# OpenVisualCloud/SVT-VP9

Hardware: AMD Instinct MI355X
Metric: hot-path frames/sec (+ Mpixels/sec): block-level DSP path (picture analysis + ME + inter prediction from reconstructed references + DCT/quant/recon + deblock + reference padding), 3840x2160p60 yuv420p enc-mode 8; no mode decision, no entropy coding -- not encoded frames (higher is better)
Workload: dtype u8

## Files before the change

### include/svtvp9_hip.h

```cpp
#ifndef SVTVP9_HIP_H
#define SVTVP9_HIP_H

#include <stddef.h>
#include <stdint.h>

#ifdef __cplusplus
extern "C" {
#endif

typedef enum svt_hip_status {
    SVT_HIP_OK                 = 0,
    SVT_HIP_ERR_BAD_PARAMETER  = -1,
    SVT_HIP_ERR_NO_RESOURCES   = -2,
    SVT_HIP_ERR_DEVICE         = -3,
    SVT_HIP_ERR_UNSUPPORTED    = -4
} svt_hip_status;

typedef struct svt_hip_ctx svt_hip_ctx;


#define SVT_ME_PU_COUNT 85
#define SVT_SB_SIZE 64

typedef struct svt_plane {
// ... 63 lines not shown

typedef struct svt_me_picture_config {
    int32_t pic_width, pic_height;
    int32_t enc_mode;
    int32_t tune;
    int32_t frame_rate;
    int32_t num_ref_lists;
    int32_t temporal_layer_index;
    int32_t hierarchical_levels;
    int32_t is_used_as_reference;
    int32_t same_ref_poc;
    int32_t rate_control_mode;
} svt_me_picture_config;

int32_t svt_hip_me_params_derive(svt_me_params *p, const svt_me_picture_config *cfg);

int32_t svt_hip_me_params_preset(svt_me_params *p, int32_t pic_width, int32_t pic_height, int32_t enc_mode,
                                 int32_t tune, int32_t num_ref_lists, int32_t temporal_layer_index,
                                 int32_t hierarchical_levels);

int32_t svt_hip_me_kernel_instance(const svt_me_params *p);
int32_t svt_hip_me_last_instance(const svt_hip_ctx *ctx);
int32_t svt_hip_me_lds_bytes(const svt_me_params *p, int32_t compact);
int32_t svt_hip_ctx_set_intra_workgroups(svt_hip_ctx *ctx, int32_t n);
int32_t svt_hip_ctx_warm(svt_hip_ctx *ctx);
int32_t svt_hip_ctx_warm_scratch(svt_hip_ctx *ctx, int32_t scratch_bytes);
int32_t svt_hip_me_params_same_launch(const svt_me_params *a, const svt_me_params *b);

int32_t svt_hip_ctx_create(svt_hip_ctx **ctx, int32_t device_ordinal);
int32_t svt_hip_ctx_create_on_stream(svt_hip_ctx **ctx, int32_t device_ordinal, void *hip_stream);
int32_t svt_hip_ctx_create_cu_mask(svt_hip_ctx **ctx, int32_t device, const uint32_t *cu_mask, int32_t mask_words);
void *svt_hip_ctx_stream(svt_hip_ctx *ctx);
void    svt_hip_ctx_destroy(svt_hip_ctx *ctx);
int32_t svt_hip_ctx_synchronize(svt_hip_ctx *ctx);
const char *svt_hip_last_error(void);
float   svt_hip_last_kernel_ms(svt_hip_ctx *ctx);

int32_t svt_hip_mem_alloc(svt_hip_ctx *ctx, size_t bytes, void **d_ptr);
void    svt_hip_mem_free(svt_hip_ctx *ctx, void *d_ptr);
int32_t svt_hip_mem_upload_2d(svt_hip_ctx *ctx, void *d_dst, size_t dst_stride, const void *src, size_t src_stride, size_t width_bytes,
                              size_t rows);
int32_t svt_hip_mem_download(svt_hip_ctx *ctx, void *dst, const void *d_src, size_t bytes);
int32_t svt_hip_mem_upload_2d_async(svt_hip_ctx *ctx, void *d_dst, size_t dst_stride, const void *src, size_t src_stride, size_t width_bytes,
                                    size_t rows);
int32_t svt_hip_mem_upload_planes_async(svt_hip_ctx *ctx, int32_t n_planes, void *const *d_dst, const size_t *dst_stride, const void *const *src,
                                        const size_t *src_stride, const size_t *width_bytes, const size_t *rows);
// ... 625 lines not shown
```

### svt-vp9_amd/binding.py

```python
import ctypes as C
import os

import numpy as np

HERE = os.path.dirname(os.path.abspath(__file__))
LIB_PATH = os.environ.get("SVT_HIP_LIB") or os.path.join(HERE, "libsvtvp9_hip.so")

SVT_ME_PU_COUNT = 85


class Plane(C.Structure):
    _fields_ = [("buf", C.c_void_p), ("stride", C.c_int32), ("origin_x", C.c_int32), ("origin_y", C.c_int32),
                ("width", C.c_int32), ("height", C.c_int32)]


class PaPicture(C.Structure):
    _fields_ = [("full", Plane), ("quarter", Plane), ("sixteenth", Plane)]


class MeParams(C.Structure):
    _fields_ = [(n, C.c_uint8) for n in (
        "num_ref_lists", "temporal_layer_index", "hierarchical_levels", "enable_hme_flag",
        "enable_hme_level_0_flag", "enable_hme_level_1_flag", "enable_hme_level_2_flag", "cu8x8_mode",
        "cu16x16_mode", "same_ref_poc", "rate_control_mode", "fractional_search_method",
# ... 210 lines not shown
OIS_BLOCK_DTYPE = np.dtype([("sad", "<u4"), ("uv_sad", "<u4"), ("mode", "u1"), ("uv_mode", "u1"), ("pad", "u1", (2,))])
assert OIS_BLOCK_DTYPE.itemsize == 12
OIS_PER_SB = 340
OIS_NONE = 0xFFFFFFFF

EXPORTS = [
    "svt_hip_sb_count", "svt_hip_input_resolution", "svt_hip_me_params_derive", "svt_hip_me_params_preset", "svt_hip_ctx_create", "svt_hip_ctx_create_on_stream", "svt_hip_ctx_create_cu_mask", "svt_hip_ctx_stream",
    "svt_hip_ctx_destroy", "svt_hip_ctx_synchronize", "svt_hip_last_error", "svt_hip_last_kernel_ms",
    "svt_hip_mem_alloc", "svt_hip_mem_free", "svt_hip_mem_upload_2d", "svt_hip_mem_upload_2d_async", "svt_hip_mem_upload_planes_async", "svt_hip_mem_download", "svt_hip_mem_set",
    "svt_hip_ctx_marker_record", "svt_hip_ctx_marker_query", "svt_hip_ctx_marker_wait", "svt_hip_minigop_split",
    "svt_hip_me_picture_device", "svt_hip_me_batch_device", "svt_hip_me_batch_layers_device", "svt_hip_me_picture", "svt_hip_sad_loop_batch_device",
    "svt_hip_me_zz_sad_device", "svt_hip_me_similar_collocated", "svt_hip_me_sb_stats_device", "svt_hip_pa_prepare_batch_device", "svt_hip_pa_mean_variance_device",
    "svt_hip_quant_tables_init", "svt_hip_tq_batch_device", "svt_hip_tq_batch_dist_device", "svt_hip_tq_rd_batch_device", "svt_hip_tq_rd_batch_multi_device", "svt_hip_rate_scan4x4_table", "svt_hip_tq_batch", "svt_hip_lf_thresh_init", "svt_hip_lf_level_from_q",
    "svt_hip_lf_frame_device", "svt_hip_lf_batch_device", "svt_hip_lf_frame", "svt_hip_lf_build_masks",
    "svt_hip_inter_pred_batch_device", "svt_hip_inter_pred_frame", "svt_hip_ref_pad_batch_device", "svt_hip_coeff_rate_batch_device", "svt_hip_coeff_rate_batch",
    "svt_hip_gop_owner", "svt_hip_gop_assign", "svt_hip_minigop_reference_source", "svt_hip_device_set_create", "svt_hip_device_set_size",
    "svt_hip_device_set_ctx", "svt_hip_device_set_destroy", "svt_hip_ref_handoff_device",
    "svt_ivf_stream_header", "svt_ivf_packetize",
    "svt_hip_tq_blocks_from_grid", "svt_hip_vp9_iscan_tables", "svt_hip_vp9_qindex_from_qp", "svt_hip_vp9_dc_step", "svt_hip_vp9_ac_step",
    "svt_hip_quant_tables_for_qindex", "svt_hip_encdec_flags_derive", "svt_hip_encdec_work_create", "svt_hip_encdec_work_destroy",
    "svt_hip_encdec_batch_device", "svt_hip_encdec_intra_device", "svt_hip_md_intra_default_device", "svt_hip_encdec_work_status", "svt_hip_encdec_work_download", "svt_hip_md_default_batch_device",
    "svt_hip_md_default_picture", "svt_hip_lf_build_masks_device", "svt_hip_ctx_wait_marker", "svt_hip_host_alloc", "svt_hip_host_free",
    "svt_hip_mem_download_2d_async", "svt_hip_mem_copy_2d_device", "svt_hip_encdec_work_set_stage_hook", "svt_hip_me_params_same_launch", "svt_hip_me_kernel_instance", "svt_hip_ctx_set_intra_workgroups", "svt_hip_ctx_warm", "svt_hip_ctx_warm_scratch", "svt_hip_lf_reserve",
    "svt_hip_me_last_instance", "svt_hip_me_lds_bytes", "svt_hip_vp9_layer_qindex", "svt_hip_mem_upload_2d_direct", "svt_hip_mem_upload_wait", "svt_hip_host_unregister_all", "svt_hip_host_registry_retain", "svt_hip_host_registry_release",
    "svt_hip_intra_search_device", "svt_hip_md_intra_search_device", "svt_hip_md_intra_search_picture",
    "svt_hip_pa_noise_params_derive", "svt_hip_pa_noise_batch_device", "svt_hip_pa_histogram_batch_device", "svt_hip_pa_chroma_mean_batch_device",
    "svt_hip_vp9_scan_tables", "svt_hip_tokenize_blocks_device", "svt_hip_tokenize_blocks", "svt_hip_tokenize_blocks_host", "svt_hip_tokenize_batch_device", "svt_hip_tokenize_picture",
    "svt_hip_tokenize_capacity",
    "svt_hip_boolcode_set_tables", "svt_hip_boolcode_batch_device", "svt_hip_boolcode", "svt_hip_boolcode_host", "svt_hip_boolcode_capacity", "svt_hip_boolcode_bools_capacity",
    "svt_hip_boolcode_geometry",
    "svt_hip_modes_set_tables", "svt_hip_modes_kf_batch_device", "svt_hip_modes_kf_picture", "svt_hip_modes_segments", "svt_hip_modes_bools_capacity",
    "svt_hip_modes_inter_set_tables", "svt_hip_modes_inter_batch_device", "svt_hip_modes_inter_picture", "svt_hip_modes_inter_bools_capacity",
    "svt_hip_mvrefs_batch_device", "svt_hip_mvrefs_picture",
    "svt_hip_md_inter_modes_batch_device", "svt_hip_md_inter_modes_picture",
    "svt_hip_frame_header_host", "svt_hip_frame_show_existing_host", "svt_hip_frame_batch_device", "svt_hip_frame_assemble_host", "svt_hip_frame_geometry",
]

_lib = None


def load():
    global _lib
    if _lib is None:
        if not os.path.exists(LIB_PATH):
            raise RuntimeError(f"{LIB_PATH} not built: run `python -c 'import __graft_entry__ as g; g.build()'`")
        try:
            import torch
# ... 84 lines not shown
```

### svt-vp9_amd/csrc/intra_kernel.hip

```cpp
#include <hip/hip_runtime.h>
#include "tq_core.h"
#include "encdec_core.h"
#include "intra_pred.h"
#include <stdlib.h>

namespace {

struct intra_pic_dev {
    const uint8_t *src[3];
    uint8_t       *pred[3];
    uint8_t       *rec[3];
    int32_t        src_stride[2], pred_stride[2], rec_stride[2];
    const svt_lf_mode_info *mi;
    int32_t        mi_stride, mi_rows, mi_cols, sb_cols, sb_rows, width, height;
    const svt_quant_tables *qtabs;
    const int16_t *iscan;
    uint32_t       iscan_off[16];
    int16_t       *qcoeff, *dqcoeff;
    uint16_t      *eob_map;
    uint8_t       *nz;
    int32_t       *sync;
    int32_t       *status;
    int32_t        mixed;
};

#ifdef INTRA_FENCES
#define INTRA_WT false
#define INTRA_LD(p) (*(p))
#else
#define INTRA_WT true
#define INTRA_LD(p) __hip_atomic_load((p), __ATOMIC_RELAXED, __HIP_MEMORY_SCOPE_AGENT)
#endif
#ifdef INTRA_PROF
__device__ unsigned long long g_intra_fine[8];
#define IPF(k) do { if (lane == 0) { const unsigned long long n_ = __builtin_amdgcn_s_memtime(); atomicAdd(&g_intra_fine[k], n_ - ipf_t); ipf_t = n_; } } while (0)
#else
#define IPF(k) ((void)0)
#endif
#define INTRA_TILE_DW  (2 * 32 * 33)
#define INTRA_SLICE_DW (INTRA_TILE_DW + 128 / 4)
#define INTRA_W        4
template <int N>
__device__ __forceinline__ int intra_block(const intra_pic_dev &P, int plane, int x0, int y0, int mode, int sb, int32_t *lds, int have_right = 0) {
    const int lane = (int)__lane_id(), c = plane ? 1 : 0;
    int32_t *const tile = lds + __builtin_amdgcn_readfirstlane((int)threadIdx.x >> 6) * INTRA_SLICE_DW;
    uint8_t *const edge = (uint8_t *)(tile + INTRA_TILE_DW);
    const int rs = P.rec_stride[c];
    uint8_t  *rp = P.rec[plane];
    const int have_left = x0 > 0, have_top = y0 > 0;
    const bool active = lane < N;
    const int  i = lane % N;
#ifdef INTRA_PROF
    unsigned long long ipf_t = __builtin_amdgcn_s_memtime();
#endif
    uint32_t   srow[N / 4], prow[N / 4];
    constexpr uintptr_t AM = N >= 16 ? 15 : N - 1;
    {
        const uint8_t *sp = P.src[plane] + (size_t)(y0 + i) * P.src_stride[c] + x0;
        _Pragma("unroll") for (int q = 0; q < N / 4; q++) srow[q] = 0u;
        if (active) row_load<N>(sp, ((uintptr_t)sp & AM) == 0, srow);
    }
    {
// ... 11 lines not shown
        if (lane == 0) edge[32] = have_top ? (have_left ? INTRA_LD(&rp[(size_t)(y0 - 1) * rs + x0 - 1]) : (uint8_t)129) : (uint8_t)127;
    }
    tq_block_sync();
    IPF(0);
    intra_pred_row<N>(edge, mode, i, have_left, have_top, prow);
    {
        if (active && P.pred[plane]) {
            uint8_t *pp = P.pred[plane] + (size_t)(y0 + i) * P.pred_stride[c] + x0;
            row_store<N>(pp, ((uintptr_t)pp & AM) == 0, prow);
        }
    }
    IPF(1);
    svt_tq_block k;
    k.src_off = k.pred_off = 0;
    k.recon_off = (uint32_t)y0 * (uint32_t)rs + (uint32_t)x0;
    k.coeff_off = (uint32_t)sb * SVT_SB_COEFFS + (plane == 0 ? 0u : plane == 1 ? 4096u : 5120u) + svt_zorder4((x0 & (plane ? 31 : 63)) >> 2, (y0 & (plane ? 31 : 63)) >> 2) * 16u;
    k.tx_size = (uint8_t)txcfg<N>::size;
    k.tx_type = (uint8_t)((plane == 0 && N < 32) ? intra_tx_type(mode) : 0);
    k.iscan_off = P.iscan_off[k.tx_size * 4 + k.tx_type];
    k.src_stride = k.pred_stride = 0; k.recon_stride = (uint16_t)rs;
    k.qtab = (uint8_t)c; k.do_recon = 1; k.partial32 = 0; k.pad_[0] = 0;
    const int pw4 = (plane ? P.width >> 1 : P.width) >> 2, w4 = P.width >> 2, h4 = P.height >> 2;
    const int eo = plane == 0 ? 0 : w4 * h4 + (plane == 2 ? (w4 >> 1) * (h4 >> 1) : 0);
    int32_t *t = tile + (lane / N) * (N * (N + 1));
    const int eob = tq_block_body<N, false, false, INTRA_WT>(k, active, i, t, srow, prow, P.qtabs, P.iscan, P.qcoeff, P.dqcoeff,
                                                   P.eob_map + eo + (y0 >> 2) * pw4 + (x0 >> 2), nullptr, nullptr, nullptr, nullptr, nullptr, rp);
    IPF(2);
    __builtin_amdgcn_fence(__ATOMIC_SEQ_CST, "workgroup");
    tq_block_sync();
    IPF(3);
    return __builtin_amdgcn_readfirstlane(eob);
}

#ifndef INTRA_WAVES_PER_EU
#define INTRA_WAVES_PER_EU 4
#endif
#ifdef INTRA_NUM_VGPR
__attribute__((amdgpu_num_vgpr(INTRA_NUM_VGPR)))
#endif
__global__ __launch_bounds__(64 * INTRA_W) __attribute__((amdgpu_waves_per_eu(INTRA_WAVES_PER_EU, INTRA_WAVES_PER_EU))) void svt_intra_kernel(const intra_pic_dev P, const int n_workers) {
    constexpr int W = INTRA_W;
    __shared__ int32_t s_lds[W * INTRA_SLICE_DW];
    const int wave = __builtin_amdgcn_readfirstlane((int)threadIdx.x >> 6);
    if ((int)blockIdx.x * W + wave >= n_workers) return;
    const int lane = (int)__lane_id(), c_cols = (P.width + 15) >> 4, c_rows = (P.height + 15) >> 4, n_cell = c_cols * c_rows;
    __builtin_amdgcn_s_setprio(3);
#ifdef INTRA_PROF
  unsigned long long pf[5] = {0, 0, 0, 0, 0}, pf_n = 0;
// ... 150 lines not shown
```

### svt-vp9_amd/csrc/tq_core.h

```cpp
#ifndef SVT_TQ_CORE_H
#define SVT_TQ_CORE_H
#include <hip/hip_runtime.h>
#include "svt_ctx.h"
#include "txfm1d.h"
#include "encdec_core.h"
#include "rate_core.h"

namespace {

struct tq_rate_args {
    const svt_rate_tables *T;
    const int16_t         *scan;
    int32_t               *bits;
};

struct tq_dev_count {
    const int32_t *p; int s;
    const uint32_t *pos; const uint8_t *geom; int geom_stride; const uint32_t *iscan_off; int sb_cols;
};

struct tq_walk { int per_xcd, first, step, base; };
__device__ __forceinline__ tq_walk tq_walk_of(int ngroups) {
    tq_walk w;
    w.per_xcd = (ngroups + 7) >> 3;
// ... 2 lines not shown
    w.step    = (int)(gridDim.x >> 3);
    return w;
}

#define TQ_DPP(v, ctrl) __builtin_amdgcn_update_dpp(0, (int)(v), (ctrl), 0xf, 0xf, false)
template <int N> __device__ __forceinline__ int tq_lanes_max(int v) {
    int o;
    o = TQ_DPP(v, 0xB1); v = o > v ? o : v;
    o = TQ_DPP(v, 0x4E); v = o > v ? o : v;
    if constexpr (N >= 8) { o = TQ_DPP(v, 0x141); v = o > v ? o : v; }
    if constexpr (N >= 16) { o = TQ_DPP(v, 0x140); v = o > v ? o : v; }
    if constexpr (N >= 32) { o = __builtin_amdgcn_ds_swizzle(v, 0x401F); v = o > v ? o : v; }
    return v;
}
template <int N> __device__ __forceinline__ uint32_t tq_lanes_sum(uint32_t v) {
    v += (uint32_t)TQ_DPP(v, 0xB1);
    v += (uint32_t)TQ_DPP(v, 0x4E);
    if constexpr (N >= 8) v += (uint32_t)TQ_DPP(v, 0x141);
    if constexpr (N >= 16) v += (uint32_t)TQ_DPP(v, 0x140);
    if constexpr (N >= 32) v += (uint32_t)__builtin_amdgcn_ds_swizzle((int)v, 0x401F);
    return v;
}

template <int N, bool RATE> constexpr int tq_threads() { return 256; }

template <int N> struct txcfg;
template <> struct txcfg<4> { static constexpr int size = SVT_TX_4X4, shift = 4; };
template <> struct txcfg<8> { static constexpr int size = SVT_TX_8X8, shift = 5; };
template <> struct txcfg<16> { static constexpr int size = SVT_TX_16X16, shift = 6; };
template <> struct txcfg<32> { static constexpr int size = SVT_TX_32X32, shift = 6; };

template <int N> __device__ __forceinline__ void fwd1d_hybrid(const int32_t *v, int32_t *o, bool adst) {
    if constexpr (N == 4) {
        if (adst) tx_fadst4(v, o);
        else { tx_fdct4(v, o); _Pragma("unroll") for (int i = 0; i < 4; i++) o[i] = (int16_t)o[i]; }
    } else if constexpr (N == 8) {
        if (adst) tx_adst8(v, o);
        else { tx_fdct8(v, o, 1); _Pragma("unroll") for (int i = 0; i < 8; i++) o[i] = (int16_t)o[i]; }
    } else {
        int32_t oa[16], od[16];
        if (adst) tx_adst16(v, oa);
        else { tx_fdct16(v, od); _Pragma("unroll") for (int i = 0; i < 16; i++) od[i] = (int16_t)od[i]; }
        _Pragma("unroll") for (int i = 0; i < 16; i++) o[i] = adst ? oa[i] : od[i];
    }
}
template <int N> __device__ __forceinline__ void fwd1d_dct(const int32_t *v, int32_t *o) {
    if constexpr (N == 4) tx_fdct4(v, o);
// ... 13 lines not shown
}

template <int N> __device__ __forceinline__ void row_load(const uint8_t *p, bool vec, uint32_t *w) {
    if constexpr (N == 4) { w[0] = *(const uint32_t *)p; }
    else if constexpr (N == 8) {
        if (vec) { const uint2 t = *(const uint2 *)p; w[0] = t.x; w[1] = t.y; }
        else { w[0] = ((const uint32_t *)p)[0]; w[1] = ((const uint32_t *)p)[1]; }
    } else {
        if (vec) { _Pragma("unroll") for (int j = 0; j < N / 16; j++) { const uint4 t = ((const uint4 *)p)[j]; w[4 * j] = t.x; w[4 * j + 1] = t.y; w[4 * j + 2] = t.z; w[4 * j + 3] = t.w; } }
        else { _Pragma("unroll") for (int j = 0; j < N / 4; j++) w[j] = ((const uint32_t *)p)[j]; }
    }
}
template <int N> __device__ __forceinline__ void row_store(uint8_t *p, bool vec, const uint32_t *w) {
    if constexpr (N == 4) { *(uint32_t *)p = w[0]; }
    else if constexpr (N == 8) {
        if (vec) *(uint2 *)p = make_uint2(w[0], w[1]);
        else { ((uint32_t *)p)[0] = w[0]; ((uint32_t *)p)[1] = w[1]; }
    } else {
        if (vec) { _Pragma("unroll") for (int j = 0; j < N / 16; j++) ((uint4 *)p)[j] = make_uint4(w[4 * j], w[4 * j + 1], w[4 * j + 2], w[4 * j + 3]); }
        else { _Pragma("unroll") for (int j = 0; j < N / 4; j++) ((uint32_t *)p)[j] = w[j]; }
    }
}

__device__ __forceinline__ void tq_block_sync() {
    __builtin_amdgcn_fence(__ATOMIC_RELEASE, "wavefront");
    __builtin_amdgcn_wave_barrier();
    __builtin_amdgcn_fence(__ATOMIC_ACQUIRE, "wavefront");
}

__device__ __forceinline__ int clamp16(int v) { return v < -32768 ? -32768 : v > 32767 ? 32767 : v; }
__device__ __forceinline__ uint8_t clip_add(int d, int t) { int v = d + t; return (uint8_t)(v < 0 ? 0 : v > 255 ? 255 : v); }

template <int N, bool RATE, bool DIST, bool WT = false>
__device__ __forceinline__ int tq_block_body(const svt_tq_block &k, const bool active, const int i, int32_t *t, const uint32_t (&srow)[N / 4],
                                              const uint32_t (&prow)[N / 4], const svt_quant_tables *__restrict__ qtabs, const int16_t *__restrict__ iscan_all,
                                              int16_t *__restrict__ qcoeff, int16_t *__restrict__ dqcoeff, uint16_t *eob_slot, uint64_t *dist_slot, int32_t *bits_slot,
                                              const svt_rate_tables *rate_T, const uint32_t *s_tc, const int16_t *s_scan, uint8_t *recon_base) {
    constexpr int LS = N + 1;
    constexpr int SCAN_T = 3 * N * N + 2;
    const int  tx_type = (N == 32) ? SVT_DCT_DCT : k.tx_type;
    const bool col_adst = tx_type == SVT_ADST_DCT || tx_type == SVT_ADST_ADST;
    const bool row_adst = tx_type == SVT_DCT_ADST || tx_type == SVT_ADST_ADST;

    int32_t  v[N], o[N];
    _Pragma("unroll") for (int cc = 0; cc < N; cc++)
        t[i * LS + cc] = (int16_t)((int)((srow[cc >> 2] >> (8 * (cc & 3))) & 0xff) - (int)((prow[cc >> 2] >> (8 * (cc & 3))) & 0xff));
    _Pragma("unroll") for (int r = 0; r < N; r++) v[r] = t[r * LS + i];
    if (tx_type == SVT_DCT_DCT) {
        _Pragma("unroll") for (int r = 0; r < N; r++) v[r] *= (N == 4 ? 16 : 4);
        if (N == 4 && i == 0 && v[0]) ++v[0];
        fwd1d_dct<N>(v, o);
        _Pragma("unroll") for (int kk = 0; kk < N; kk++) {
            int32_t m;
            if constexpr (N == 32) m = (o[kk] + 1 + (o[kk] > 0)) >> 2;
            else m = (int16_t)o[kk];
            if (N == 32 && k.partial32 && kk >= 16) m = 0;
            t[kk * LS + i] = m;
        }
    } else {
        _Pragma("unroll") for (int r = 0; r < N; r++) v[r] = (int16_t)(v[r] * (N == 4 ? 16 : 4));
        if (N == 4 && i == 0 && v[0]) v[0] = (int16_t)(v[0] + 1);
        if constexpr (N < 32) fwd1d_hybrid<N>(v, o, col_adst);
        _Pragma("unroll") for (int kk = 0; kk < N; kk++)
            t[kk * LS + i] = (N == 16) ? (int16_t)((o[kk] + 1 + (o[kk] < 0)) >> 2) : (int16_t)o[kk];
    }
    tq_block_sync();
    _Pragma("unroll") for (int kk = 0; kk < N; kk++) v[kk] = t[i * LS + kk];
    int32_t c[N];
    if (tx_type == SVT_DCT_DCT) {
        if constexpr (N == 16) { _Pragma("unroll") for (int kk = 0; kk < N; kk++) v[kk] = (v[kk] + 1) >> 2; }
        fwd1d_dct<N>(v, o);
        _Pragma("unroll") for (int kk = 0; kk < N; kk++) {
            if constexpr (N == 4) c[kk] = (int16_t)(((int16_t)o[kk] + 1) >> 2);
            else if constexpr (N == 8) c[kk] = (int16_t)((int16_t)o[kk] / 2);
            else if constexpr (N == 16) c[kk] = (int16_t)o[kk];
            else c[kk] = (int16_t)((o[kk] + 1 + (o[kk] < 0)) >> 2);
        }
        if (N == 32 && k.partial32) {
            _Pragma("unroll") for (int kk = 0; kk < N; kk++) if (i >= 16 || kk >= 16) c[kk] = 0;
        }
    } else {
        if constexpr (N < 32) fwd1d_hybrid<N>(v, o, row_adst);
        _Pragma("unroll") for (int kk = 0; kk < N; kk++) {
            const int32_t tt = o[kk];
            c[kk] = (N == 4) ? (int16_t)((tt + 1) >> 2) : (N == 8) ? (int16_t)((tt + (tt < 0)) >> 1) : (int16_t)tt;
        }
    }
    svt_quant_tables q;
    {
        const uint32_t *qp = (const uint32_t *)(qtabs + k.qtab);
// ... 68 lines not shown
        const int16_t *sc = s_scan + tx_type * SCAN_T;
        int bits = rate_positions<N>((const int16_t *)t, sc, sc + N * N, s_tc + (ptype * 2 + inter) * RATE_SLICE, rate_T, i, eob, N * N,
                                     txcfg<N>::size, ctx0);
        bits = (int)tq_lanes_sum<N>((uint32_t)bits);
        if (active && i == 0) *bits_slot = bits;
    }
    if (k.do_recon) {
    int32_t res[N];
    _Pragma("unroll") for (int r = 0; r < N; r++) res[r] = 0;
    const bool dct_path = tx_type == SVT_DCT_DCT;
    bool dc_only = false;
    int  nrows = N;
    if (dct_path) {
        if (N == 4) dc_only = eob <= 1;
        else dc_only = eob == 1;
        if (N == 8) nrows = eob <= 12 ? 4 : 8;
        if (N == 16) nrows = eob <= 10 ? 4 : eob <= 38 ? 8 : 16;
        if (N == 32) nrows = eob <= 34 ? 8 : eob <= 135 ? 16 : 32;
    }
    tq_block_sync();
    if (eob != 0 && !dc_only) {
        if (i < nrows) inv1d<N>(dq, o, row_adst);
        else { _Pragma("unroll") for (int kk = 0; kk < N; kk++) o[kk] = 0; }
        _Pragma("unroll") for (int kk = 0; kk < N; kk++) t[i * LS + kk] = (int16_t)o[kk];
    } else if (eob != 0 && i == 0) {
        t[0] = dq[0];
    }
    tq_block_sync();
    if (eob != 0 && !dc_only) {
        _Pragma("unroll") for (int r = 0; r < N; r++) v[r] = t[r * LS + i];
        inv1d<N>(v, o, col_adst);
        _Pragma("unroll") for (int r = 0; r < N; r++) res[r] = ((int16_t)o[r] + (1 << (txcfg<N>::shift - 1))) >> txcfg<N>::shift;
    } else if (eob != 0) {
        int32_t d = tx_rsw((int16_t)t[0] * TX_C16);
        d = tx_rsw(d * TX_C16);
        const int32_t a1 = (d + (1 << (txcfg<N>::shift - 1))) >> txcfg<N>::shift;
        _Pragma("unroll") for (int r = 0; r < N; r++) res[r] = a1;
    }
    _Pragma("unroll") for (int r = 0; r < N; r++) t[r * LS + i] = res[r];
    if (active && recon_base) {
        uint8_t *d = recon_base + k.recon_off + (size_t)i * k.recon_stride;
        uint32_t rw[N / 4];
        _Pragma("unroll") for (int q = 0; q < N / 4; q++) {
            uint32_t w = 0;
            _Pragma("unroll") for (int b = 0; b < 4; b++)
                w |= (uint32_t)clip_add((int)((prow[q] >> (8 * b)) & 0xff), t[i * LS + 4 * q + b]) << (8 * b);
            rw[q] = w;
        }
        if constexpr (WT) {
            _Pragma("unroll") for (int q = 0; q < N / 4; q++) __hip_atomic_store((uint32_t *)d + q, rw[q], __ATOMIC_RELAXED, __HIP_MEMORY_SCOPE_AGENT);
        } else row_store<N>(d, ((uintptr_t)d & (N >= 16 ? 15 : N - 1)) == 0, rw);
    }
    }
    return eob;
}

}
#endif
```

### svt-vp9_amd/csrc/tq_kernel.hip

```cpp
#include <hip/hip_runtime.h>
#include <type_traits>
#include "tq_core.h"

namespace {

__device__ __forceinline__ void tq_loads_landed() { __builtin_amdgcn_s_waitcnt(0x0F70);  }

template <int N, bool RATE, bool DIST> constexpr bool tq_pipelined() { return N < 16 && !RATE; }

template <int N, bool RATE, bool DIST>
__global__ __launch_bounds__(256) __attribute__((amdgpu_waves_per_eu(N == 32 ? (RATE ? 3 : 4) : 1))) void svt_tq_kernel(const uint8_t *__restrict__ src, const uint8_t *__restrict__ pred,
                                                     uint8_t *__restrict__ recon, const svt_tq_block *__restrict__ blocks,
                                                     int n_blocks, const svt_quant_tables *__restrict__ qtabs,
                                                     const int16_t *__restrict__ iscan_all, int16_t *__restrict__ qcoeff,
                                                     int16_t *__restrict__ dqcoeff, uint16_t *__restrict__ eob_out,
                                                     uint64_t *__restrict__ dist_out, tq_rate_args ra, const uint8_t *const *__restrict__ recon_set, tq_dev_count dc) {
    if (dc.p) {
        const int o = dc.p[dc.s];
        n_blocks = dc.p[4 + dc.s];
        blocks += o; eob_out += o;
        if (dc.pos) dc.pos += o;
        if (dist_out) dist_out += 2 * o;
        if constexpr (RATE) ra.bits += o;
    }
    constexpr int NT  = tq_threads<N, RATE>();
    constexpr int BPW = NT / N;
    constexpr int LS  = N + 1;
    __shared__ int32_t tile[BPW][N * LS];
    __shared__ uint32_t s_tc[RATE ? 4 * RATE_SLICE : 1];
    constexpr int SCAN_T = 3 * N * N + 2, SCAN_N = N == 32 ? 3 * N * N : 4 * SCAN_T;
    __shared__ int16_t s_scan[RATE ? SCAN_N : 2];
    if constexpr (RATE) {
        const uint32_t *g = &ra.T->token_costs[txcfg<N>::size][0][0][0][0][0][0];
        for (int j = threadIdx.x; j < 4 * RATE_SLICE; j += NT) s_tc[j] = g[j];
        const uint32_t *gs = (const uint32_t *)(ra.scan + rate_scan_offset(txcfg<N>::size, 0));
        for (int j = threadIdx.x; j < SCAN_N / 2; j += NT) ((uint32_t *)s_scan)[j] = gs[j];
        __syncthreads();
    }
    const int lb  = threadIdx.x / N;
    const int i   = threadIdx.x % N;
    const tq_walk wk = tq_walk_of((n_blocks + BPW - 1) / BPW);
    auto in_walk = [&](int gj) { return gj < wk.per_xcd && (wk.base + gj) * BPW < n_blocks; };
    auto code_of = [&](int gj) { const int blk = (wk.base + gj) * BPW + lb; return dc.pos[blk < n_blocks ? blk : 0]; };
    auto block_of = [&](auto POS, int gj, uint32_t pc, svt_tq_block &k) {
        const int blk = (wk.base + gj) * BPW + lb;
        if constexpr (decltype(POS)::value)
            svt_tq_block_from_pos(pc, txcfg<N>::size, (const svt_tq_pic_geom *)(dc.geom + (size_t)svt_tq_pos_pic(pc) * dc.geom_stride), dc.iscan_off, dc.sb_cols, &k);
        else k = blocks[blk < n_blocks ? blk : 0];
    };
    auto rows_of = [&](int gj, const svt_tq_block &k, uint32_t (&srow)[N / 4], uint32_t (&prow)[N / 4]) {
        _Pragma("unroll") for (int q = 0; q < N / 4; q++) { srow[q] = 0u; prow[q] = 0u; }
        if ((wk.base + gj) * BPW + lb >= n_blocks) return;
        const uint8_t *sp = src + k.src_off + (size_t)i * k.src_stride;
        const uint8_t *pp = pred + k.pred_off + (size_t)i * k.pred_stride;
        constexpr uintptr_t AM = N >= 16 ? 15 : N - 1;
        row_load<N>(sp, ((uintptr_t)sp & AM) == 0, srow); row_load<N>(pp, ((uintptr_t)pp & AM) == 0, prow);
    };
    auto body_of = [&](int gj, const svt_tq_block &k, const uint32_t (&srow)[N / 4], const uint32_t (&prow)[N / 4]) {
        const int  blk = (wk.base + gj) * BPW + lb;
        const bool active = blk < n_blocks;
        int32_t *bits_slot = nullptr;
        if constexpr (RATE) bits_slot = ra.bits + blk;
        tq_block_body<N, RATE, DIST>(k, active, i, tile[lb], srow, prow, qtabs, iscan_all, qcoeff, dqcoeff, eob_out + blk, dist_out ? dist_out + 2 * blk : nullptr, bits_slot,
                                     ra.T, s_tc, s_scan, recon_set ? (uint8_t *)recon_set[(k.pad_[0] >> 4) & 7] : recon);
        tq_block_sync();
    };
    int gj = wk.first;
    if constexpr (!tq_pipelined<N, RATE, DIST>()) {
        for (; gj < wk.per_xcd; gj += wk.step) {
            const int grp = wk.base + gj;
            if (grp * BPW >= n_blocks) break;
            const int blk = grp * BPW + lb;
            const bool active = blk < n_blocks;
            svt_tq_block k;
            if (dc.pos) {
                const uint32_t pc = dc.pos[active ? blk : 0];
                svt_tq_block_from_pos(pc, txcfg<N>::size, (const svt_tq_pic_geom *)(dc.geom + (size_t)svt_tq_pos_pic(pc) * dc.geom_stride), dc.iscan_off, dc.sb_cols, &k);
            } else if (active) k = blocks[blk];
            else { k = blocks[0]; }
            int32_t *t = tile[lb];
            uint32_t srow[N / 4], prow[N / 4];
            {
                const uint8_t *sp = src + k.src_off + (size_t)i * k.src_stride;
                const uint8_t *pp = pred + k.pred_off + (size_t)i * k.pred_stride;
                constexpr uintptr_t AM = N >= 16 ? 15 : N - 1;
                _Pragma("unroll") for (int q = 0; q < N / 4; q++) { srow[q] = 0u; prow[q] = 0u; }
                if (active) { row_load<N>(sp, ((uintptr_t)sp & AM) == 0, srow); row_load<N>(pp, ((uintptr_t)pp & AM) == 0, prow); }
            }
            int32_t *bits_slot = nullptr;
            if constexpr (RATE) bits_slot = ra.bits + blk;
            tq_block_body<N, RATE, DIST>(k, active, i, t, srow, prow, qtabs, iscan_all, qcoeff, dqcoeff, eob_out + blk, dist_out ? dist_out + 2 * blk : nullptr, bits_slot,
                                         ra.T, s_tc, s_scan, recon_set ? (uint8_t *)recon_set[(k.pad_[0] >> 4) & 7] : recon);
            tq_block_sync();
        }
    } else {
        auto walk = [&](auto POS) {
            constexpr bool P = decltype(POS)::value;
            bool     have0 = in_walk(gj), have1 = have0 && in_walk(gj + wk.step);
            uint32_t pc0 = 0u, pc1 = 0u, s0[N / 4], p0[N / 4];
            if constexpr (P) { if (have0) pc0 = code_of(gj); if (have1) pc1 = code_of(gj + wk.step); }
            if (have0) { svt_tq_block k; block_of(POS, gj, pc0, k); rows_of(gj, k, s0, p0); }
            while (have0) {
                const int  g1 = gj + wk.step, g2 = g1 + wk.step;
                const bool have2 = have1 && in_walk(g2);
                uint32_t   pc2 = 0u, s1[N / 4], p1[N / 4];
                svt_tq_block k, kn;
                block_of(POS, gj, pc0, k);
                block_of(POS, have1 ? g1 : gj, have1 ? pc1 : pc0, kn);
                tq_loads_landed();
                if (have1) rows_of(g1, kn, s1, p1);
                else { _Pragma("unroll") for (int q = 0; q < N / 4; q++) { s1[q] = 0u; p1[q] = 0u; } }
                if constexpr (P) { if (have2) pc2 = code_of(g2); }
                body_of(gj, k, s0, p0);
                _Pragma("unroll") for (int q = 0; q < N / 4; q++) { s0[q] = s1[q]; p0[q] = p1[q]; }
// ... 255 lines not shown
            block_of(POS, have1 ? g1 : gj, have1 ? pc1 : pc0, kn);
            tq_loads_landed();
            if (have1) tq_lane_rows<N>(kn, src, pred, s1, p1);
            if constexpr (P) { if (have2) pc2 = dc.pos[blk_of(g2)]; }
            tq_lane_block<N, RATE, DIST>(k, blk_of(gj), s0, p0, recon, qtabs, iscan_all, qcoeff, dqcoeff, eob_out, dist_out, ra, s_tc, s_vc, recon_set);
            _Pragma("unroll") for (int r = 0; r < N; r++) { _Pragma("unroll") for (int q = 0; q < N / 4; q++) { s0[r][q] = s1[r][q]; p0[r][q] = p1[r][q]; } }
            pc0 = pc1; pc1 = pc2; gj = g1; have0 = have1; have1 = have2;
        }
    };
    if (dc.pos) walk(std::true_type{}); else walk(std::false_type{});
}

int tq_grid(svt_hip_ctx *ctx, int ngroups, int per_2cu, int size) {
    static const struct grid_env { int v[4]; } env = [] {
        grid_env g = {{0, 0, 0, 0}};
        if (const char *e = getenv("SVT_HIP_TQ_GRID")) sscanf(e, "%d,%d,%d,%d", &g.v[0], &g.v[1], &g.v[2], &g.v[3]);
        return g;
    }();
    const int per_xcd = (ngroups + 7) / 8, cap = env.v[size] > 0 ? (env.v[size] + 7) / 8 : (ctx->cu_count * per_2cu + 15) / 16;
    return 8 * (per_xcd < cap ? per_xcd : cap);
}

constexpr int TQ_PER_2CU = 12;
constexpr int TQ_PER_2CU_ENC[4] = {1, 4, 4, 4};

template <int N, bool RATE, bool DIST = true>
hipError_t launch_tq(svt_hip_ctx *ctx, const uint8_t *src, const uint8_t *pred, uint8_t *recon, const svt_tq_block *blocks, int n,
                     const svt_quant_tables *q, const int16_t *iscan, int16_t *qc, int16_t *dqc, uint16_t *eob, uint64_t *dist, tq_rate_args ra,
                     const uint8_t *const *recon_set, tq_dev_count dc = {nullptr, 0, nullptr, nullptr, 0, nullptr, 0}, int per_2cu = TQ_PER_2CU) {
    if (n <= 0) return hipSuccess;
    if constexpr (N == 4) {
        hipLaunchKernelGGL((svt_tq_lane_kernel<N, RATE, DIST>), dim3(tq_grid(ctx, (n + 255) / 256, per_2cu, 0)), dim3(256), 0, ctx->stream, src, pred, recon, blocks, n, q,
                           iscan, qc, dqc, eob, dist, ra, recon_set, dc);
        return hipGetLastError();
    } else {
        constexpr int NT = tq_threads<N, RATE>(), BPW = NT / N;
        hipLaunchKernelGGL((svt_tq_kernel<N, RATE, DIST>), dim3(tq_grid(ctx, (n + BPW - 1) / BPW, per_2cu, txcfg<N>::size)), dim3(NT), 0, ctx->stream, src, pred, recon, blocks, n, q,
                           iscan, qc, dqc, eob, dist, ra, recon_set, dc);
        return hipGetLastError();
    }
}

int32_t tq_stage_recon_set(svt_hip_ctx *ctx, uint8_t *const *recon_set, int n_set, const uint8_t *const **d_set) {
    void *h = nullptr, *d = nullptr;
    if (svt_ctx_stage(ctx, 8 * sizeof(void *), &h, &d)) return svt_set_error(SVT_HIP_ERR_NO_RESOURCES, "tq: descriptor buffers");
    for (int i = 0; i < 8; i++) ((uint8_t **)h)[i] = i < n_set ? recon_set[i] : nullptr;
    HIP_TRY(svt_ctx_stage_send(ctx, 8 * sizeof(void *)));
    *d_set = (const uint8_t *const *)d;
    return SVT_HIP_OK;
}

template <bool RATE>
int32_t tq_launch_all(svt_hip_ctx *ctx, const uint8_t *d_src, const uint8_t *d_pred, uint8_t *d_recon, const svt_tq_block *d_blocks,
                      const int32_t size_count[4], const svt_quant_tables *d_qtabs, const int16_t *d_iscan, int16_t *d_qcoeff,
                      int16_t *d_dqcoeff, uint16_t *d_eob, uint64_t *d_dist, tq_rate_args ra, uint8_t *const *recon_set = nullptr, int n_set = 0) {
    HIP_TRY(hipSetDevice(ctx->device));
    const uint8_t *const *d_set = nullptr;
    if (recon_set)
        if (const int32_t e = tq_stage_recon_set(ctx, recon_set, n_set, &d_set)) return e;
    svt_ctx_timer timer(ctx);
// ... 3 lines not shown
    auto at = [&](int o) { tq_rate_args r = ra; if (r.bits) r.bits += o; return r; };
    rc = launch_tq<4, RATE>(ctx, d_src, d_pred, d_recon, d_blocks + off, size_count[0], d_qtabs, d_iscan, d_qcoeff, d_dqcoeff, d_eob + off, d_dist ? d_dist + 2 * off : nullptr, at(off), d_set);
    off += size_count[0];
    if (rc == hipSuccess) rc = launch_tq<8, RATE>(ctx, d_src, d_pred, d_recon, d_blocks + off, size_count[1], d_qtabs, d_iscan, d_qcoeff, d_dqcoeff, d_eob + off, d_dist ? d_dist + 2 * off : nullptr, at(off), d_set);
    off += size_count[1];
    if (rc == hipSuccess) rc = launch_tq<16, RATE>(ctx, d_src, d_pred, d_recon, d_blocks + off, size_count[2], d_qtabs, d_iscan, d_qcoeff, d_dqcoeff, d_eob + off, d_dist ? d_dist + 2 * off : nullptr, at(off), d_set);
    off += size_count[2];
    if (rc == hipSuccess) rc = launch_tq<32, RATE>(ctx, d_src, d_pred, d_recon, d_blocks + off, size_count[3], d_qtabs, d_iscan, d_qcoeff, d_dqcoeff, d_eob + off, d_dist ? d_dist + 2 * off : nullptr, at(off), d_set);
    HIP_TRY(rc);
    HIP_TRY(timer.end());
    return SVT_HIP_OK;
}
}

int32_t svt_tq_launch_device_lists(svt_hip_ctx *ctx, const uint8_t *d_src, const uint8_t *d_pred, uint8_t *const *recon_set, int n_set,
                                   const svt_tq_block *d_blocks, const int32_t cap[4], const int32_t *d_off_cnt, const svt_quant_tables *d_qtabs,
                                   const int16_t *d_iscan, int16_t *d_qcoeff, int16_t *d_dqcoeff, uint16_t *d_eob, uint64_t *d_dist,
                                   const uint32_t *d_pos, const void *d_geom, int geom_stride, const uint32_t *d_iscan_off, int sb_cols) {
    HIP_TRY(hipSetDevice(ctx->device));
    const uint8_t *const *d_set = nullptr;
    if (const int32_t e = tq_stage_recon_set(ctx, recon_set, n_set, &d_set)) return e;
    const tq_rate_args none = {nullptr, nullptr, nullptr};
    hipError_t rc = hipSuccess;
#define TQ_DEV(N, S, D) launch_tq<N, false, D>(ctx, d_src, d_pred, nullptr, d_blocks, cap[S], d_qtabs, d_iscan, d_qcoeff, d_dqcoeff, d_eob, d_dist, none, d_set, tq_dev_count{d_off_cnt, S, d_pos, (const uint8_t *)d_geom, geom_stride, d_iscan_off, sb_cols}, TQ_PER_2CU_ENC[S])
    if (d_dist) {
        rc = TQ_DEV(4, 0, true);
        if (rc == hipSuccess) rc = TQ_DEV(8, 1, true);
        if (rc == hipSuccess) rc = TQ_DEV(16, 2, true);
        if (rc == hipSuccess) rc = TQ_DEV(32, 3, true);
    } else {
        rc = TQ_DEV(4, 0, false);
        if (rc == hipSuccess) rc = TQ_DEV(8, 1, false);
        if (rc == hipSuccess) rc = TQ_DEV(16, 2, false);
        if (rc == hipSuccess) rc = TQ_DEV(32, 3, false);
    }
#undef TQ_DEV
    HIP_TRY(rc);
    return SVT_HIP_OK;
}

extern "C" int32_t svt_hip_tq_batch_device(svt_hip_ctx *ctx, const uint8_t *d_src, const uint8_t *d_pred, uint8_t *d_recon,
                                           const svt_tq_block *d_blocks, const int32_t size_count[4],
                                           const svt_quant_tables *d_qtabs, const int16_t *d_iscan, int16_t *d_qcoeff,
                                           int16_t *d_dqcoeff, uint16_t *d_eob) {
    return svt_hip_tq_batch_dist_device(ctx, d_src, d_pred, d_recon, d_blocks, size_count, d_qtabs, d_iscan, d_qcoeff, d_dqcoeff, d_eob,
                                        nullptr);
}

extern "C" int32_t svt_hip_tq_batch_dist_device(svt_hip_ctx *ctx, const uint8_t *d_src, const uint8_t *d_pred, uint8_t *d_recon,
                                                const svt_tq_block *d_blocks, const int32_t size_count[4],
                                                const svt_quant_tables *d_qtabs, const int16_t *d_iscan, int16_t *d_qcoeff,
                                                int16_t *d_dqcoeff, uint16_t *d_eob, uint64_t *d_dist) {
    if (!ctx || !d_src || !d_pred || !d_blocks || !size_count || !d_qtabs || !d_iscan || !d_qcoeff || !d_dqcoeff || !d_eob)
        return svt_set_error(SVT_HIP_ERR_BAD_PARAMETER, "tq: null argument");
    if (((uintptr_t)d_qcoeff | (uintptr_t)d_dqcoeff) & 15) return svt_set_error(SVT_HIP_ERR_BAD_PARAMETER, "tq: coefficient arrays must be 16-byte aligned");
    tq_rate_args none = {nullptr, nullptr, nullptr};
    return tq_launch_all<false>(ctx, d_src, d_pred, d_recon, d_blocks, size_count, d_qtabs, d_iscan, d_qcoeff, d_dqcoeff, d_eob, d_dist, none);
}

extern "C" int32_t svt_hip_tq_rd_batch_device(svt_hip_ctx *ctx, const uint8_t *d_src, const uint8_t *d_pred, uint8_t *d_recon,
                                              const svt_tq_block *d_blocks, const int32_t size_count[4],
// ... 78 lines not shown
```

Before: 6776.

## Pack TQ transpose tiles as 16-bit pairs and shrink encode-pass workgroups

Stores the transform transpose tile in LDS as packed 16-bit pairs instead of 32-bit words, for the non-rate TQ kernels and the intra kernel. This halves LDS per block. The encode pass now launches 8x8 and 16x16 blocks with smaller workgroups (128/64 threads) and raises the per-2CU grid factor to add occupancy. The packed tile adds pack and unpack ALU work and a possible bank-conflict pattern, and it relies on intermediates fitting in int16. A helper that reports TQ LDS bytes is also added.

```diff
diff --git a/include/svtvp9_hip.h b/include/svtvp9_hip.h
--- a/include/svtvp9_hip.h
+++ b/include/svtvp9_hip.h
@@ -109,6 +109,7 @@
 int32_t svt_hip_me_kernel_instance(const svt_me_params *p);
 int32_t svt_hip_me_last_instance(const svt_hip_ctx *ctx);
 int32_t svt_hip_me_lds_bytes(const svt_me_params *p, int32_t compact);
+int32_t svt_hip_tq_lds_bytes(int32_t tx_size, int32_t encode_pass);
 int32_t svt_hip_ctx_set_intra_workgroups(svt_hip_ctx *ctx, int32_t n);
 int32_t svt_hip_ctx_warm(svt_hip_ctx *ctx);
 int32_t svt_hip_ctx_warm_scratch(svt_hip_ctx *ctx, int32_t scratch_bytes);
diff --git a/svt-vp9_amd/binding.py b/svt-vp9_amd/binding.py
--- a/svt-vp9_amd/binding.py
+++ b/svt-vp9_amd/binding.py
@@ -256,7 +256,7 @@
     "svt_hip_encdec_batch_device", "svt_hip_encdec_intra_device", "svt_hip_md_intra_default_device", "svt_hip_encdec_work_status", "svt_hip_encdec_work_download", "svt_hip_md_default_batch_device",
     "svt_hip_md_default_picture", "svt_hip_lf_build_masks_device", "svt_hip_ctx_wait_marker", "svt_hip_host_alloc", "svt_hip_host_free",
     "svt_hip_mem_download_2d_async", "svt_hip_mem_copy_2d_device", "svt_hip_encdec_work_set_stage_hook", "svt_hip_me_params_same_launch", "svt_hip_me_kernel_instance", "svt_hip_ctx_set_intra_workgroups", "svt_hip_ctx_warm", "svt_hip_ctx_warm_scratch", "svt_hip_lf_reserve",
-    "svt_hip_me_last_instance", "svt_hip_me_lds_bytes", "svt_hip_vp9_layer_qindex", "svt_hip_mem_upload_2d_direct", "svt_hip_mem_upload_wait", "svt_hip_host_unregister_all", "svt_hip_host_registry_retain", "svt_hip_host_registry_release",
+    "svt_hip_me_last_instance", "svt_hip_me_lds_bytes", "svt_hip_tq_lds_bytes","svt_hip_vp9_layer_qindex", "svt_hip_mem_upload_2d_direct", "svt_hip_mem_upload_wait", "svt_hip_host_unregister_all", "svt_hip_host_registry_retain", "svt_hip_host_registry_release",
     "svt_hip_intra_search_device", "svt_hip_md_intra_search_device", "svt_hip_md_intra_search_picture",
     "svt_hip_pa_noise_params_derive", "svt_hip_pa_noise_batch_device", "svt_hip_pa_histogram_batch_device", "svt_hip_pa_chroma_mean_batch_device",
     "svt_hip_vp9_scan_tables", "svt_hip_tokenize_blocks_device", "svt_hip_tokenize_blocks", "svt_hip_tokenize_blocks_host", "svt_hip_tokenize_batch_device", "svt_hip_tokenize_picture",
diff --git a/svt-vp9_amd/csrc/intra_kernel.hip b/svt-vp9_amd/csrc/intra_kernel.hip
--- a/svt-vp9_amd/csrc/intra_kernel.hip
+++ b/svt-vp9_amd/csrc/intra_kernel.hip
@@ -37,7 +37,7 @@
 #else
 #define IPF(k) ((void)0)
 #endif
-#define INTRA_TILE_DW  (2 * 32 * 33)
+#define INTRA_TILE_DW  (2 * 32 * 17)
 #define INTRA_SLICE_DW (INTRA_TILE_DW + 128 / 4)
 #define INTRA_W        4
 template <int N>
@@ -95,8 +95,9 @@
     k.qtab = (uint8_t)c; k.do_recon = 1; k.partial32 = 0; k.pad_[0] = 0;
     const int pw4 = (plane ? P.width >> 1 : P.width) >> 2, w4 = P.width >> 2, h4 = P.height >> 2;
     const int eo = plane == 0 ? 0 : w4 * h4 + (plane == 2 ? (w4 >> 1) * (h4 >> 1) : 0);
-    int32_t *t = tile + (lane / N) * (N * (N + 1));
-    const int eob = tq_block_body<N, false, false, INTRA_WT>(k, active, i, t, srow, prow, P.qtabs, P.iscan, P.qcoeff, P.dqcoeff,
+    static_assert((64 / N) * tq_tile_dwords<N, true>() <= INTRA_TILE_DW, "the wave's tiles fit the slice");
+    int32_t *t = tile + (lane / N) * tq_tile_dwords<N, true>();
+    const int eob = tq_block_body<N, false, false, INTRA_WT, true>(k, active, i, t, srow, prow, P.qtabs, P.iscan, P.qcoeff, P.dqcoeff,
                                                    P.eob_map + eo + (y0 >> 2) * pw4 + (x0 >> 2), nullptr, nullptr, nullptr, nullptr, nullptr, rp);
     IPF(2);
     __builtin_amdgcn_fence(__ATOMIC_SEQ_CST, "workgroup");
diff --git a/svt-vp9_amd/csrc/tq_core.h b/svt-vp9_amd/csrc/tq_core.h
--- a/svt-vp9_amd/csrc/tq_core.h
+++ b/svt-vp9_amd/csrc/tq_core.h
@@ -48,7 +48,7 @@
     return v;
 }
 
-template <int N, bool RATE> constexpr int tq_threads() { return 256; }
+template <int N, bool RATE, bool ENC = false> constexpr int tq_threads() { return (ENC && !RATE && N == 8) ? 128 : (ENC && !RATE && N == 16) ? 64 : 256; }
 
 template <int N> struct txcfg;
 template <> struct txcfg<4> { static constexpr int size = SVT_TX_4X4, shift = 4; };
@@ -108,6 +108,22 @@
     }
 }
 
+typedef int16_t __attribute__((may_alias)) tq_h16;
+template <int N, bool T16> constexpr int tq_tile_dwords() { return T16 ? N * (N / 2 + 1) : N * (N + 1); }
+template <int N, bool T16, bool ALONG_ROW> __device__ __forceinline__ void tile_put(int32_t *t, int i, const int32_t (&x)[N]) {
+    if constexpr (T16) {
+        _Pragma("unroll") for (int j = 0; j < N / 2; j++) t[i * (N / 2 + 1) + j] = (int32_t)(((uint32_t)x[2 * j] & 0xffffu) | ((uint32_t)x[2 * j + 1] << 16));
+    } else if constexpr (ALONG_ROW) { _Pragma("unroll") for (int j = 0; j < N; j++) t[i * (N + 1) + j] = x[j]; }
+    else { _Pragma("unroll") for (int j = 0; j < N; j++) t[j * (N + 1) + i] = x[j]; }
+}
+template <int N, bool T16, bool ALONG_ROW> __device__ __forceinline__ void tile_get(const int32_t *t, int i, int32_t (&x)[N]) {
+    if constexpr (T16) {
+        const tq_h16 *h = (const tq_h16 *)t;
+        _Pragma("unroll") for (int j = 0; j < N; j++) x[j] = h[j * (N + 2) + i];
+    } else if constexpr (ALONG_ROW) { _Pragma("unroll") for (int j = 0; j < N; j++) x[j] = t[j * (N + 1) + i]; }
+    else { _Pragma("unroll") for (int j = 0; j < N; j++) x[j] = t[i * (N + 1) + j]; }
+}
+
 __device__ __forceinline__ void tq_block_sync() {
     __builtin_amdgcn_fence(__ATOMIC_RELEASE, "wavefront");
     __builtin_amdgcn_wave_barrier();
@@ -117,12 +133,12 @@
 __device__ __forceinline__ int clamp16(int v) { return v < -32768 ? -32768 : v > 32767 ? 32767 : v; }
 __device__ __forceinline__ uint8_t clip_add(int d, int t) { int v = d + t; return (uint8_t)(v < 0 ? 0 : v > 255 ? 255 : v); }
 
-template <int N, bool RATE, bool DIST, bool WT = false>
+template <int N, bool RATE, bool DIST, bool WT = false, bool T16 = false>
 __device__ __forceinline__ int tq_block_body(const svt_tq_block &k, const bool active, const int i, int32_t *t, const uint32_t (&srow)[N / 4],
                                               const uint32_t (&prow)[N / 4], const svt_quant_tables *__restrict__ qtabs, const int16_t *__restrict__ iscan_all,
                                               int16_t *__restrict__ qcoeff, int16_t *__restrict__ dqcoeff, uint16_t *eob_slot, uint64_t *dist_slot, int32_t *bits_slot,
                                               const svt_rate_tables *rate_T, const uint32_t *s_tc, const int16_t *s_scan, uint8_t *recon_base) {
-    constexpr int LS = N + 1;
+    static_assert(!(RATE && T16), "the rate walk reads raster coefficients from a 32-bit tile");
     constexpr int SCAN_T = 3 * N * N + 2;
     const int  tx_type = (N == 32) ? SVT_DCT_DCT : k.tx_type;
     const bool col_adst = tx_type == SVT_ADST_DCT || tx_type == SVT_ADST_ADST;
@@ -130,8 +146,9 @@
 
     int32_t  v[N], o[N];
     _Pragma("unroll") for (int cc = 0; cc < N; cc++)
-        t[i * LS + cc] = (int16_t)((int)((srow[cc >> 2] >> (8 * (cc & 3))) & 0xff) - (int)((prow[cc >> 2] >> (8 * (cc & 3))) & 0xff));
-    _Pragma("unroll") for (int r = 0; r < N; r++) v[r] = t[r * LS + i];
+        o[cc] = (int16_t)((int)((srow[cc >> 2] >> (8 * (cc & 3))) & 0xff) - (int)((prow[cc >> 2] >> (8 * (cc & 3))) & 0xff));
+    tile_put<N, T16, true>(t, i, o);
+    tile_get<N, T16, true>(t, i, v);
     if (tx_type == SVT_DCT_DCT) {
         _Pragma("unroll") for (int r = 0; r < N; r++) v[r] *= (N == 4 ? 16 : 4);
         if (N == 4 && i == 0 && v[0]) ++v[0];
@@ -141,17 +158,18 @@
             if constexpr (N == 32) m = (o[kk] + 1 + (o[kk] > 0)) >> 2;
             else m = (int16_t)o[kk];
             if (N == 32 && k.partial32 && kk >= 16) m = 0;
-            t[kk * LS + i] = m;
+            o[kk] = m;
         }
     } else {
         _Pragma("unroll") for (int r = 0; r < N; r++) v[r] = (int16_t)(v[r] * (N == 4 ? 16 : 4));
         if (N == 4 && i == 0 && v[0]) v[0] = (int16_t)(v[0] + 1);
         if constexpr (N < 32) fwd1d_hybrid<N>(v, o, col_adst);
         _Pragma("unroll") for (int kk = 0; kk < N; kk++)
-            t[kk * LS + i] = (N == 16) ? (int16_t)((o[kk] + 1 + (o[kk] < 0)) >> 2) : (int16_t)o[kk];
-    }
+            o[kk] = (N == 16) ? (int16_t)((o[kk] + 1 + (o[kk] < 0)) >> 2) : (int16_t)o[kk];
+    }
+    tile_put<N, T16, false>(t, i, o);
     tq_block_sync();
-    _Pragma("unroll") for (int kk = 0; kk < N; kk++) v[kk] = t[i * LS + kk];
+    tile_get<N, T16, false>(t, i, v);
     int32_t c[N];
     if (tx_type == SVT_DCT_DCT) {
         if constexpr (N == 16) { _Pragma("unroll") for (int kk = 0; kk < N; kk++) v[kk] = (v[kk] + 1) >> 2; }
@@ -266,29 +284,31 @@
     if (eob != 0 && !dc_only) {
         if (i < nrows) inv1d<N>(dq, o, row_adst);
         else { _Pragma("unroll") for (int kk = 0; kk < N; kk++) o[kk] = 0; }
-        _Pragma("unroll") for (int kk = 0; kk < N; kk++) t[i * LS + kk] = (int16_t)o[kk];
+        _Pragma("unroll") for (int kk = 0; kk < N; kk++) o[kk] = (int16_t)o[kk];
+        tile_put<N, T16, true>(t, i, o);
     } else if (eob != 0 && i == 0) {
         t[0] = dq[0];
     }
     tq_block_sync();
     if (eob != 0 && !dc_only) {
-        _Pragma("unroll") for (int r = 0; r < N; r++) v[r] = t[r * LS + i];
+        tile_get<N, T16, true>(t, i, v);
         inv1d<N>(v, o, col_adst);
         _Pragma("unroll") for (int r = 0; r < N; r++) res[r] = ((int16_t)o[r] + (1 << (txcfg<N>::shift - 1))) >> txcfg<N>::shift;
     } else if (eob != 0) {
-        int32_t d = tx_rsw((int16_t)t[0] * TX_C16);
+        int32_t d = tx_rsw(*(const tq_h16 *)t * TX_C16);
         d = tx_rsw(d * TX_C16);
         const int32_t a1 = (d + (1 << (txcfg<N>::shift - 1))) >> txcfg<N>::shift;
         _Pragma("unroll") for (int r = 0; r < N; r++) res[r] = a1;
     }
-    _Pragma("unroll") for (int r = 0; r < N; r++) t[r * LS + i] = res[r];
+    tile_put<N, T16, false>(t, i, res);
+    tile_get<N, T16, false>(t, i, res);
     if (active && recon_base) {
         uint8_t *d = recon_base + k.recon_off + (size_t)i * k.recon_stride;
         uint32_t rw[N / 4];
         _Pragma("unroll") for (int q = 0; q < N / 4; q++) {
             uint32_t w = 0;
             _Pragma("unroll") for (int b = 0; b < 4; b++)
-                w |= (uint32_t)clip_add((int)((prow[q] >> (8 * b)) & 0xff), t[i * LS + 4 * q + b]) << (8 * b);
+                w |= (uint32_t)clip_add((int)((prow[q] >> (8 * b)) & 0xff), res[4 * q + b]) << (8 * b);
             rw[q] = w;
         }
         if constexpr (WT) {
diff --git a/svt-vp9_amd/csrc/tq_kernel.hip b/svt-vp9_amd/csrc/tq_kernel.hip
--- a/svt-vp9_amd/csrc/tq_kernel.hip
+++ b/svt-vp9_amd/csrc/tq_kernel.hip
@@ -8,8 +8,10 @@
 
 template <int N, bool RATE, bool DIST> constexpr bool tq_pipelined() { return N < 16 && !RATE; }
 
-template <int N, bool RATE, bool DIST>
-__global__ __launch_bounds__(256) __attribute__((amdgpu_waves_per_eu(N == 32 ? (RATE ? 3 : 4) : 1))) void svt_tq_kernel(const uint8_t *__restrict__ src, const uint8_t *__restrict__ pred,
+template <bool RATE> constexpr bool tq_tile16() { return !RATE; }
+
+template <int N, bool RATE, bool DIST, int NT = 256>
+__global__ __launch_bounds__(NT) __attribute__((amdgpu_waves_per_eu(N == 32 ? (RATE ? 3 : 4) : 1))) void svt_tq_kernel(const uint8_t *__restrict__ src, const uint8_t *__restrict__ pred,
                                                      uint8_t *__restrict__ recon, const svt_tq_block *__restrict__ blocks,
                                                      int n_blocks, const svt_quant_tables *__restrict__ qtabs,
                                                      const int16_t *__restrict__ iscan_all, int16_t *__restrict__ qcoeff,
@@ -23,19 +25,22 @@
         if (dist_out) dist_out += 2 * o;
         if constexpr (RATE) ra.bits += o;
     }
-    constexpr int NT  = tq_threads<N, RATE>();
-    constexpr int BPW = NT / N;
-    constexpr int LS  = N + 1;
-    __shared__ int32_t tile[BPW][N * LS];
-    __shared__ uint32_t s_tc[RATE ? 4 * RATE_SLICE : 1];
-    constexpr int SCAN_T = 3 * N * N + 2, SCAN_N = N == 32 ? 3 * N * N : 4 * SCAN_T;
-    __shared__ int16_t s_scan[RATE ? SCAN_N : 2];
+    static_assert(NT % 64 == 0 && 64 % N == 0, "whole waves of whole blocks");
+    constexpr bool T16 = tq_tile16<RATE>();
+    constexpr int  BPW = NT / N;
+    __shared__ int32_t tile[BPW][tq_tile_dwords<N, T16>()];
+    const uint32_t *s_tc = nullptr;
+    const int16_t  *s_scan = nullptr;
     if constexpr (RATE) {
+        __shared__ uint32_t tc[4 * RATE_SLICE];
+        constexpr int SCAN_T = 3 * N * N + 2, SCAN_N = N == 32 ? 3 * N * N : 4 * SCAN_T;
+        __shared__ int16_t scan[SCAN_N];
         const uint32_t *g = &ra.T->token_costs[txcfg<N>::size][0][0][0][0][0][0];
-        for (int j = threadIdx.x; j < 4 * RATE_SLICE; j += NT) s_tc[j] = g[j];
+        for (int j = threadIdx.x; j < 4 * RATE_SLICE; j += NT) tc[j] = g[j];
         const uint32_t *gs = (const uint32_t *)(ra.scan + rate_scan_offset(txcfg<N>::size, 0));
-        for (int j = threadIdx.x; j < SCAN_N / 2; j += NT) ((uint32_t *)s_scan)[j] = gs[j];
+        for (int j = threadIdx.x; j < SCAN_N / 2; j += NT) ((uint32_t *)scan)[j] = gs[j];
         __syncthreads();
+        s_tc = tc; s_scan = scan;
     }
     const int lb  = threadIdx.x / N;
     const int i   = threadIdx.x % N;
@@ -61,7 +66,7 @@
         const bool active = blk < n_blocks;
         int32_t *bits_slot = nullptr;
         if constexpr (RATE) bits_slot = ra.bits + blk;
-        tq_block_body<N, RATE, DIST>(k, active, i, tile[lb], srow, prow, qtabs, iscan_all, qcoeff, dqcoeff, eob_out + blk, dist_out ? dist_out + 2 * blk : nullptr, bits_slot,
+        tq_block_body<N, RATE, DIST, false, T16>(k, active, i, tile[lb], srow, prow, qtabs, iscan_all, qcoeff, dqcoeff, eob_out + blk, dist_out ? dist_out + 2 * blk : nullptr, bits_slot,
                                      ra.T, s_tc, s_scan, recon_set ? (uint8_t *)recon_set[(k.pad_[0] >> 4) & 7] : recon);
         tq_block_sync();
     };
@@ -89,7 +94,7 @@
             }
             int32_t *bits_slot = nullptr;
             if constexpr (RATE) bits_slot = ra.bits + blk;
-            tq_block_body<N, RATE, DIST>(k, active, i, t, srow, prow, qtabs, iscan_all, qcoeff, dqcoeff, eob_out + blk, dist_out ? dist_out + 2 * blk : nullptr, bits_slot,
+            tq_block_body<N, RATE, DIST, false, T16>(k, active, i, t, srow, prow, qtabs, iscan_all, qcoeff, dqcoeff, eob_out + blk, dist_out ? dist_out + 2 * blk : nullptr, bits_slot,
                                          ra.T, s_tc, s_scan, recon_set ? (uint8_t *)recon_set[(k.pad_[0] >> 4) & 7] : recon);
             tq_block_sync();
         }
@@ -391,9 +396,9 @@
 }
 
 constexpr int TQ_PER_2CU = 12;
-constexpr int TQ_PER_2CU_ENC[4] = {1, 4, 4, 4};
-
-template <int N, bool RATE, bool DIST = true>
+constexpr int TQ_PER_2CU_ENC[4] = {1, 8, 10, 4};
+
+template <int N, bool RATE, bool DIST = true, bool ENC = false>
 hipError_t launch_tq(svt_hip_ctx *ctx, const uint8_t *src, const uint8_t *pred, uint8_t *recon, const svt_tq_block *blocks, int n,
                      const svt_quant_tables *q, const int16_t *iscan, int16_t *qc, int16_t *dqc, uint16_t *eob, uint64_t *dist, tq_rate_args ra,
                      const uint8_t *const *recon_set, tq_dev_count dc = {nullptr, 0, nullptr, nullptr, 0, nullptr, 0}, int per_2cu = TQ_PER_2CU) {
@@ -403,8 +408,8 @@
                            iscan, qc, dqc, eob, dist, ra, recon_set, dc);
         return hipGetLastError();
     } else {
-        constexpr int NT = tq_threads<N, RATE>(), BPW = NT / N;
-        hipLaunchKernelGGL((svt_tq_kernel<N, RATE, DIST>), dim3(tq_grid(ctx, (n + BPW - 1) / BPW, per_2cu, txcfg<N>::size)), dim3(NT), 0, ctx->stream, src, pred, recon, blocks, n, q,
+        constexpr int NT = tq_threads<N, RATE, ENC>(), BPW = NT / N;
+        hipLaunchKernelGGL((svt_tq_kernel<N, RATE, DIST, NT>), dim3(tq_grid(ctx, (n + BPW - 1) / BPW, per_2cu, txcfg<N>::size)), dim3(NT), 0, ctx->stream, src, pred, recon, blocks, n, q,
                            iscan, qc, dqc, eob, dist, ra, recon_set, dc);
         return hipGetLastError();
     }
@@ -454,7 +459,7 @@
     if (const int32_t e = tq_stage_recon_set(ctx, recon_set, n_set, &d_set)) return e;
     const tq_rate_args none = {nullptr, nullptr, nullptr};
     hipError_t rc = hipSuccess;
-#define TQ_DEV(N, S, D) launch_tq<N, false, D>(ctx, d_src, d_pred, nullptr, d_blocks, cap[S], d_qtabs, d_iscan, d_qcoeff, d_dqcoeff, d_eob, d_dist, none, d_set, tq_dev_count{d_off_cnt, S, d_pos, (const uint8_t *)d_geom, geom_stride, d_iscan_off, sb_cols}, TQ_PER_2CU_ENC[S])
+#define TQ_DEV(N, S, D) launch_tq<N, false, D, true>(ctx, d_src, d_pred, nullptr, d_blocks, cap[S], d_qtabs, d_iscan, d_qcoeff, d_dqcoeff, d_eob, d_dist, none, d_set, tq_dev_count{d_off_cnt, S, d_pos, (const uint8_t *)d_geom, geom_stride, d_iscan_off, sb_cols}, TQ_PER_2CU_ENC[S])
     if (d_dist) {
         rc = TQ_DEV(4, 0, true);
         if (rc == hipSuccess) rc = TQ_DEV(8, 1, true);
@@ -469,6 +474,21 @@
 #undef TQ_DEV
     HIP_TRY(rc);
     return SVT_HIP_OK;
+}
+
+extern "C" int32_t svt_hip_tq_lds_bytes(int32_t tx_size, int32_t encode_pass) {
+    auto bytes = [&](auto n) {
+        constexpr int N = decltype(n)::value;
+        const int nt = encode_pass ? tq_threads<N, false, true>() : tq_threads<N, false, false>();
+        return (int32_t)((nt / N) * tq_tile_dwords<N, tq_tile16<false>()>() * (int)sizeof(int32_t));
+    };
+    switch (tx_size) {
+    case SVT_TX_4X4: return 0;
+    case SVT_TX_8X8: return bytes(std::integral_constant<int, 8>{});
+    case SVT_TX_16X16: return bytes(std::integral_constant<int, 16>{});
+    case SVT_TX_32X32: return bytes(std::integral_constant<int, 32>{});
+    }
+    return svt_set_error(SVT_HIP_ERR_BAD_PARAMETER, "tq_lds_bytes: bad transform size");
 }
 
 extern "C" int32_t svt_hip_tq_batch_device(svt_hip_ctx *ctx, const uint8_t *d_src, const uint8_t *d_pred, uint8_t *d_recon,
```

Result: no change. 6765 (-0.2%).
